# yzqin/s4g-release

Hardware: AMD Instinct MI355X
Metric: scenes/sec (25.6k-pt clouds) end-to-end grasp inference (higher is better)
Workload: dtype f32 (f16x2 split)

## Files before the change

### s4g_release_amd/csrc/mlp_common.h

```cpp
#pragma once
#include "s4g_common.h"

namespace s4g {

typedef float f32x16 __attribute__((ext_vector_type(16)));
typedef __bf16 bf16x8 __attribute__((ext_vector_type(8)));
typedef _Float16 f16x8 __attribute__((ext_vector_type(8)));
typedef _Float16 f16x2 __attribute__((ext_vector_type(2)));

__device__ __forceinline__ uint32_t cvt_pk_bf16(float lo, float hi) {
  uint32_t r;
  asm("v_cvt_pk_bf16_f32 %0, %1, %2" : "=v"(r) : "v"(lo), "v"(hi));
  return r;
}


__device__ __forceinline__ uint32_t pack_h2(float a, float b) {
  f16x2 v;
  v.x = (_Float16)a;
  v.y = (_Float16)b;
  return __builtin_bit_cast(uint32_t, v);
}

__device__ __forceinline__ void split_quad_h2(float x0, float x1, float x2, float x3, float s0, float s1, float s2, float s3,
// ... 55 lines not shown

__device__ __forceinline__ float amax_rows(const float* __restrict__ slots, int lane, int p_lo, int p_hi,
                                           int rps) {
  const int s0 = rps > 0 ? p_lo / rps : 0, s1 = rps > 0 ? p_hi / rps : 0;
  float m = amax_slots(slots + (size_t)s0 * 64, lane);
  for (int sc = s0 + 1; sc <= s1; ++sc) m = fmaxf(m, amax_slots(slots + (size_t)sc * 64, lane));
  return m;
}
__device__ __forceinline__ void amax_publish(uint32_t* __restrict__ slots, uint32_t wm, int slot, int p_lo,
                                             int p_hi, int rps) {
  const int s0 = rps > 0 ? p_lo / rps : 0, s1 = rps > 0 ? p_hi / rps : 0;
  for (int sc = s0; sc <= s1; ++sc) atomicMax(slots + (size_t)sc * 64 + (slot & 63), wm);
}


typedef float f32x4 __attribute__((ext_vector_type(4)));
__device__ __forceinline__ float4 nt_load4(const float* p) {
  const f32x4 v = __builtin_nontemporal_load(reinterpret_cast<const f32x4*>(p));
  return make_float4(v.x, v.y, v.z, v.w);
}

struct WRef {
  __amdgpu_buffer_rsrc_t r;
  uint32_t off;
};
__device__ __forceinline__ WRef wref(const void* base, size_t off) {
  return WRef{__builtin_amdgcn_make_buffer_rsrc(const_cast<void*>(base), 0, 0x7FFFFFFF, 0x00020000), (uint32_t)off};
}
__device__ __forceinline__ WRef operator+(const WRef& w, size_t bytes) { return WRef{w.r, w.off + (uint32_t)bytes}; }
__device__ __forceinline__ uint4 wref_load(const WRef& w, uint32_t lane_off, uint32_t byte_off) {
  return __builtin_bit_cast(uint4, __builtin_amdgcn_raw_buffer_load_b128(w.r, (int)lane_off, (int)(w.off + byte_off), 0));
}

template <int PL>
__device__ __forceinline__ f32x16 chain_mfma(const uint4 a, const uint4 b, const f32x16 c) {
  if constexpr (PL == 2)
    return __builtin_amdgcn_mfma_f32_32x32x16_f16(__builtin_bit_cast(f16x8, a), __builtin_bit_cast(f16x8, b), c, 0, 0, 0);
  else
    return __builtin_amdgcn_mfma_f32_32x32x16_bf16(__builtin_bit_cast(bf16x8, a), __builtin_bit_cast(bf16x8, b), c, 0, 0, 0);
}

}
```

### s4g_release_amd/csrc/mlp_gemm.hip

```cpp
#include <stdlib.h>

#include "mlp_common.h"

#include <type_traits>

#ifndef S4G_CHAIN_ABLATE
#define S4G_CHAIN_ABLATE 0
#endif

namespace s4g {


constexpr int GM_BM = 128;
constexpr int GM_BN = 128;
constexpr int GM_BK = 32;
constexpr int GM_LDS = 36;
constexpr int GM_THREADS = 256;

enum { LOAD_PLAIN = 0, LOAD_GATHER = 1, LOAD_INTERP = 2, LOAD_GATHER_MLP1 = 3, LOAD_GATHER_ADD = 4,
       LOAD_INTERP_ADD = 5, LOAD_CHANNEL_FIRST = 6,
       LOAD_REL_MLP1 = 64,
       LOAD_ADD_MFMA0 = 65 };
enum { EPI_STORE = 0, EPI_MAX = 1, EPI_CHANNEL_FIRST = 2, EPI_MAX_CF = 3 };

struct GemmParams {
  int P, Cin, Kpad, Cout, relu;
  const float* W;
  const float* bias;
  const float* A;
  int lda, a_coff, a_gcol;
  int aL;
  const int* gidx;
  const float* feat;
  const float* xyz;
  const float* ctr;
  int Cf, N, M, K;
  int nscenes;
  const float4* mlp1;
  const float4* rel4;
  const int* seg4;
  const int* seg_rows;
  float* out2;
  int ldc2, split_n;
  uint32_t* out_amax2;
  const int* nidx;
  const float* nw;
  const float* sparse;
  const float* dense;
  int C2, C1, N2, N1;
  float* out;
  int ldc, c_coff, c_gcol;
  int w_gstride, b_gstride;
  float* cf_ptr[4];
  int cf_start[5];
  int cf_sigmoid_from;
// ... 882 lines not shown
    const unsigned sb_ = gridDim.x >= 1024 ? blockIdx.x - gridDim.x / 2 : blockIdx.x;    \
    if (threadIdx.x == 0 && sb_ < 512u && blockIdx.y == 0)                                 \
      g_chain_stamps[sb_ * 16 + (i)] = __builtin_amdgcn_s_memtime();                      \
  } while (0)
#else
#define S4G_STAMP(i)
#endif
constexpr int GF_RING_F16X2 = 2;
#ifndef S4G_CHAIN_RING1
#define S4G_CHAIN_RING1 2
#endif
#ifndef S4G_CHAIN_BF16_NRB
#define S4G_CHAIN_BF16_NRB 4
#endif

template <int LOADER, int EPI2, int RW, int KC, int PL>
__global__ __launch_bounds__(RW == 8 ? 512 : 256, (PL == 1 && RW != 8 && S4G_CHAIN_BF16_NRB == 2) ? 3 : 2) void mlp_chain_kernel(const GemmParams p) {
  constexpr int GF_RING = PL == 2 ? GF_RING_F16X2 : S4G_CHAIN_RING1;
  constexpr int NRB = PL == 1 ? S4G_CHAIN_BF16_NRB : 2, WROWS = 32 * NRB;
  constexpr int CW = RW == 8 ? 8 : 4 / RW, RWN = RW == 8 ? 1 : RW;
  constexpr int BM = WROWS * RWN, K = 64 * CW, NW = RWN * CW;
  constexpr int RS = 8 * NW, RPT = BM / RS;
  constexpr int astr = K + 8, aplane = BM * astr, KS = K >> 4;
  extern __shared__ __attribute__((aligned(16))) float smemf[];
  uint16_t* Ah = reinterpret_cast<uint16_t*>(smemf);
  float* scr = reinterpret_cast<float*>(Ah + PL * aplane);
  const int g = blockIdx.y;

  const int t = threadIdx.x;
  const int lane = t & 63;
  const int wave = t >> 6;

  constexpr bool ADD0 = LOADER == LOAD_ADD_MFMA0;
  constexpr bool ADD_BOUNDS = LOADER == LOAD_GATHER_ADD || LOADER == LOAD_INTERP_ADD || ADD0;
  constexpr bool MFMA0 = LOADER == LOAD_REL_MLP1;
  static_assert(!(MFMA0 || ADD0) || (PL == 2 && KC == 1), "phase 0 on the matrix cores: f16x2, one panel");
  static_assert(!ADD0 || EPI2 == EPI_MAX, "a wave's 64 rows are one centroid's neighbours");
  constexpr bool SEGMAX = (LOADER == LOAD_GATHER_MLP1 || MFMA0) && EPI2 == EPI_MAX;
  const int tile = blockIdx.x;
  const int p0 = tile * BM;
  bool seg_scene = false;
  if constexpr (SEGMAX) {
    if (p.seg_rows) {
      const int sc = p0 / p.rps;
      const int nrows = p.seg_rows[sc];
      if (p0 - sc * p.rps >= nrows) return;
      seg_scene = nrows < p.rps;
    }
  }
  const int p_hi = min(p0 + BM, p.P) - 1;
  const int am_s0 = p.rps > 0 ? p0 / p.rps : 0, am_s1 = p.rps > 0 ? p_hi / p.rps : 0;
  float am_v1 = 0.f, am_v2 = 0.f;
  if (PL == 2 && p.a_amax) am_v1 = p.a_amax[(size_t)am_s0 * 64 + lane];
  if (PL == 2 && p.a_amax2) am_v2 = p.a_amax2[(size_t)am_s0 * 64 + lane];

  const int wr = wave / CW, wc = wave % CW;
  const int li = lane & 31, lh = lane >> 5;
  const int wc_u = __builtin_amdgcn_readfirstlane(wc);
  const uint32_t wf_lane = (uint32_t)lane * 16u;
  constexpr size_t cb_stride = (size_t)KS * PL * 1024;
  constexpr size_t strip_stride = (size_t)CW * 2 * cb_stride;
  constexpr int kchunks = KC;
  const size_t cbs1 = (size_t)kchunks * cb_stride;
  const WRef w1 = wref(p.Wfrag + (size_t)g * p.Cout * p.Kpad16 * PL, (size_t)(wc_u * 2) * cbs1);
  const bool tri = p.Wfrag3 != nullptr;
  const WRef wmid = wref(p.Wfrag2 + (size_t)g * p.Cout2 * K * PL, (size_t)(wc_u * 2) * cb_stride);
  const int CoutF = tri ? p.Cout3 : p.Cout2;
  const float* __restrict__ scF = PL == 2 ? (tri ? p.w_inv_scale3 : p.w_inv_scale2) + (size_t)g * CoutF : nullptr;
  const float* __restrict__ bgF = (tri ? p.bias3 : p.bias2) + (size_t)g * CoutF;
  const WRef w2 = tri ? wref(p.Wfrag3 + (size_t)g * CoutF * K * PL, (size_t)(wc_u * 2) * cb_stride) : wmid;
  const int nstrip2 = (CoutF + 64 * CW - 1) / (64 * CW);
  const bool active0 = wc_u * 64 < CoutF;

  uint4 ring[GF_RING][2][PL];
#pragma unroll
  for (int d = 0; d < GF_RING; ++d)
#pragma unroll
    for (int cb = 0; cb < 2; ++cb)
#pragma unroll
      for (int pl = 0; pl < PL; ++pl)
        ring[d][cb][pl] = wref_load(w1, wf_lane + pl * 1024, (uint32_t)(cb * cbs1 + (size_t)d * PL * 1024));

  S4G_STAMP(0);
  ALoader<LOADER, RPT, RS> ld;
  float4 rv0[NRB];
  float4 wv0 = f4zero();
  constexpr int NKT0 = ADD0 ? K / 32 : 1, RPT0 = ADD0 ? RPT : 1;
  float4 fa[NKT0][RPT0];
  constexpr int fstr = K + 4;
  if constexpr (ADD0) {
    const int rows_left = p.P - p0;
    const __amdgpu_buffer_rsrc_t ridx = __builtin_amdgcn_make_buffer_rsrc(
        const_cast<int*>(p.gidx + p0), 0, (rows_left < BM ? rows_left : BM) * 4, 0x00020000);
    const __amdgpu_buffer_rsrc_t rxyz = __builtin_amdgcn_make_buffer_rsrc(
        const_cast<float*>(p.xyz), 0, p.nscenes * 3 * p.N * 4, 0x00020000);
    const __amdgpu_buffer_rsrc_t rfeat = __builtin_amdgcn_make_buffer_rsrc(
        const_cast<float*>(p.feat), 0, p.nscenes * p.N * p.Cf * 4, 0x00020000);
    constexpr uint32_t OOB = 0x80000000u;
    int jr[NRB], jg[RPT];
#pragma unroll
    for (int rb = 0; rb < NRB; ++rb)
      jr[rb] = __builtin_amdgcn_raw_buffer_load_b32(ridx, (wr * WROWS + rb * 32 + li) * 4, 0, 0);
#pragma unroll
    for (int s = 0; s < RPT; ++s) jg[s] = __builtin_amdgcn_raw_buffer_load_b32(ridx, ((t >> 3) + RS * s) * 4, 0, 0);
    {
      int bw, mw;
      gather_row_bm(p.M, p.K, p0, __builtin_amdgcn_readfirstlane(wr * WROWS), bw, mw);
      bw = __builtin_amdgcn_readfirstlane(bw);
      mw = __builtin_amdgcn_readfirstlane(mw);
      const bool okw = p0 + wr * WROWS < p.P;
      float cx = 0.f, cy = 0.f, cz = 0.f;
      if (okw) {
        const float* c = p.ctr + (size_t)bw * 3 * p.M + mw;
        cx = c[0];
        cy = c[p.M];
        cz = c[2 * p.M];
      }
// ... 12 lines not shown
    for (int s = 0; s < RPT; ++s) {
      const int c64 = (RS * s) / 64 * 64;
      int bc, mc;
      gather_row_bm(p.M, p.K, p0, c64, bc, mc);
      bc = __builtin_amdgcn_readfirstlane(bc);
      rowoff[s] = p0 + c64 < p.P ? (uint32_t)((bc * p.N + jg[s]) * p.Cf + (t & 7) * 4) * 4u : OOB;
    }
    if (p.Cin >= K) {
#pragma unroll
      for (int kt = 0; kt < NKT0; ++kt)
#pragma unroll
        for (int s = 0; s < RPT; ++s)
          fa[kt][s] = __builtin_bit_cast(float4, __builtin_amdgcn_raw_buffer_load_b128(rfeat, rowoff[s] + kt * 128, 0, 0));
    } else {
#pragma unroll
      for (int kt = 0; kt < NKT0; ++kt)
#pragma unroll
        for (int s = 0; s < RPT; ++s)
          fa[kt][s] = __builtin_bit_cast(float4, __builtin_amdgcn_raw_buffer_load_b128(
                                                     rfeat, kt * 32 + (t & 7) * 4 < p.Cin ? rowoff[s] + kt * 128 : OOB, 0, 0));
    }
    const int ch = wc * 64 + lane;
    if (ch < p.Cin) wv0 = p.mlp1[ch];
  } else if constexpr (MFMA0) {
    const int rows_left = p.P - p0;
    const __amdgpu_buffer_rsrc_t rrel = __builtin_amdgcn_make_buffer_rsrc(
        const_cast<float4*>(p.rel4 + p0), 0, (rows_left < BM ? rows_left : BM) * 16, 0x00020000);
#pragma unroll
    for (int rb = 0; rb < NRB; ++rb)
      rv0[rb] = __builtin_bit_cast(float4, __builtin_amdgcn_raw_buffer_load_b128(
                                               rrel, (wr * WROWS + rb * 32 + li) * 16, 0, 0));
    const int ch = wc * 64 + lane;
    if (ch < p.Cin) wv0 = p.mlp1[ch];
  } else {
    ld.init(p, p0, g, t);
  }
  S4G_STAMP(1);
  float amax = PL == 2 ? p.a_amax_floor : 1.f;
  if (PL == 2 && p.a_amax) {
    float m = __uint_as_float(wave_max_u32(__float_as_uint(am_v1)));
    for (int sc = am_s0 + 1; sc <= am_s1; ++sc) m = fmaxf(m, amax_slots(p.a_amax + (size_t)sc * 64, lane));
    amax = ADD_BOUNDS ? amax + m : fmaxf(amax, m);
  }
  if (PL == 2 && p.a_amax2) {
    float m = __uint_as_float(wave_max_u32(__float_as_uint(am_v2)));
    for (int sc = am_s0 + 1; sc <= am_s1; ++sc) m = fmaxf(m, amax_slots(p.a_amax2 + (size_t)sc * 64, lane));
    amax = ADD_BOUNDS ? amax + m : fmaxf(amax, m);
  }
  uint32_t ex = __float_as_uint(amax) >> 23;
  ex = ex < 15u ? 15u : (ex > 240u ? 240u : ex);
  ex = __builtin_amdgcn_readfirstlane(ex);
  const float sa = PL == 2 ? __uint_as_float((268u - ex) << 23) : 1.f;
  const float inv_sa = PL == 2 ? __uint_as_float((ex - 14u) << 23) : 1.f;
  auto load_panel = [&](int kc, auto depth_tag) {
    constexpr int DEPTH = decltype(depth_tag)::value;
    const int chunk = t & 7, srow = t >> 3;
    constexpr int NKT = K / 32;
#pragma unroll
    for (int kt0 = 0; kt0 < NKT; kt0 += DEPTH) {
      float4 ra[DEPTH][RPT];
#pragma unroll
      for (int kt = 0; kt < DEPTH; ++kt)
#pragma unroll
        for (int s = 0; s < RPT; ++s) ra[kt][s] = ld.load(p, s, kc * K + (kt0 + kt) * 32 + chunk * 4, t);
#pragma unroll
      for (int kt = 0; kt < DEPTH; ++kt)
#pragma unroll
        for (int s = 0; s < RPT; ++s) {
          uint16_t* dst = Ah + (srow + RS * s) * astr + (kt0 + kt) * 32 + chunk * 4;
          if constexpr (PL == 2) {
            uint2 h, l;
            split2_h<false>(ra[kt][s], sa, h, l);
            *reinterpret_cast<uint2*>(dst) = h;
            *reinterpret_cast<uint2*>(dst + aplane) = l;
          } else {
            *reinterpret_cast<uint2*>(dst) = make_uint2(cvt_pk_bf16(ra[kt][s].x, ra[kt][s].y),
                                                        cvt_pk_bf16(ra[kt][s].z, ra[kt][s].w));
          }
        }
      if (DEPTH < NKT) __builtin_amdgcn_sched_barrier(0);
    }
  };
  const uint16_t* a_lane = Ah + (wr * WROWS + li) * astr + 8 * lh;
  float* epi_s = scr + wave * 128;
  f32x16 acc[2][NRB];
  if constexpr (MFMA0 || ADD0) {
    float m = 0.f;
#pragma unroll
    for (int rb = 0; rb < NRB; ++rb)
      m = fmaxf(m, fmaxf(fmaxf(fabsf(rv0[rb].x), fabsf(rv0[rb].y)), fabsf(rv0[rb].z)));
    uint32_t ea = wave_max_u32(__float_as_uint(m)) >> 23;
    ea = ea < 90u ? 90u : (ea > 240u ? 240u : ea);
    ea = __builtin_amdgcn_readfirstlane(ea);
    const float s_a = __uint_as_float((268u - ea) << 23), inv_a = __uint_as_float((ea - 14u) << 23);
    const float one = __uint_as_float((ea + 1u) << 23), inv_one = __uint_as_float((253u - ea) << 23);
    const float bq = wv0.w * inv_one;
    const float mw = fmaxf(fmaxf(fabsf(wv0.x), fabsf(wv0.y)), fmaxf(fabsf(wv0.z), fabsf(bq)));
    uint32_t ew = __float_as_uint(mw) >> 23;
    ew = ew < 15u ? 15u : (ew > 240u ? 240u : ew);
    const float s_w = __uint_as_float((268u - ew) << 23);
    epi_s[lane] = __uint_as_float((ew - 14u) << 23) * inv_a * (ADD0 ? 1.f : sa);
    uint32_t wh01, wl01, wh23, wl23;
    split_quad_h(wv0.x, wv0.y, wv0.z, bq, s_w, wh01, wl01, wh23, wl23);
    uint4 af0[NRB][2], bf0[2][2];
#pragma unroll
    for (int cb = 0; cb < 2; ++cb) {
      bf0[cb][0] = make_uint4(lh == cb ? wh01 : 0u, lh == cb ? wh23 : 0u, 0u, 0u);
      bf0[cb][1] = make_uint4(lh == cb ? wl01 : 0u, lh == cb ? wl23 : 0u, 0u, 0u);
    }
#pragma unroll
    for (int rb = 0; rb < NRB; ++rb) {
      const float one_r = p0 + wr * WROWS + rb * 32 + li < p.P ? one : 0.f;
      uint32_t h01, l01, h23, l23;
// ... 40 lines not shown
          }
        }
      __syncthreads();
#pragma unroll
      for (int nb = 0; nb < 2; ++nb)
#pragma unroll
        for (int j = 0; j < 4; ++j)
#pragma unroll
          for (int pb = 0; pb < NRB; ++pb) {
            uint16_t* dst = Ah + (wr * WROWS + pb * 32 + li) * astr + wc * 64 + nb * 32 + 8 * j + 4 * lh;
            uint2 h, l;
            split_quad_h(fmaxf(acc[nb][pb][4 * j], 0.f), fmaxf(acc[nb][pb][4 * j + 1], 0.f),
                         fmaxf(acc[nb][pb][4 * j + 2], 0.f), fmaxf(acc[nb][pb][4 * j + 3], 0.f), sa, h.x, l.x, h.y, l.y);
            *reinterpret_cast<uint2*>(dst) = h;
            *reinterpret_cast<uint2*>(dst + aplane) = l;
          }
    } else {
#pragma unroll
      for (int nb = 0; nb < 2; ++nb)
#pragma unroll
        for (int j = 0; j < 4; ++j) {
          const float4 f4 = *reinterpret_cast<const float4*>(epi_s + nb * 32 + 8 * j + 4 * lh);
#pragma unroll
          for (int pb = 0; pb < NRB; ++pb) {
            uint16_t* dst = Ah + (wr * WROWS + pb * 32 + li) * astr + wc * 64 + nb * 32 + 8 * j + 4 * lh;
            uint2 h, l;
            split_quad_h2(fmaxf(acc[nb][pb][4 * j], 0.f), fmaxf(acc[nb][pb][4 * j + 1], 0.f),
                          fmaxf(acc[nb][pb][4 * j + 2], 0.f), fmaxf(acc[nb][pb][4 * j + 3], 0.f), f4.x, f4.y, f4.z, f4.w,
                          h.x, l.x, h.y, l.y);
            *reinterpret_cast<uint2*>(dst) = h;
            *reinterpret_cast<uint2*>(dst + aplane) = l;
          }
        }
    }
  } else {
    if (!(S4G_CHAIN_ABLATE & 16)) load_panel(0, std::integral_constant<int, (K / 32) / (NRB / 2)>{});
  }
  S4G_STAMP(2);
  __syncthreads();
  S4G_STAMP(3);

  auto zero_acc = [&]() {
#pragma unroll
    for (int i = 0; i < 2; ++i)
#pragma unroll
      for (int j = 0; j < NRB; ++j)
#pragma unroll
        for (int r = 0; r < 16; ++r) acc[i][j][r] = 0.f;
  };
  uint4 afn[NRB][PL];
  auto prime_a = [&]() {
#pragma unroll
    for (int rb = 0; rb < NRB; ++rb)
#pragma unroll
      for (int pl = 0; pl < PL; ++pl)
        afn[rb][pl] = *reinterpret_cast<const uint4*>(a_lane + pl * aplane + rb * 32 * astr);
  };

#define S4G_F2_STRIP(SWAPPED, ZFIRST, wcur, cbs_cur, wnext, cbs_next)                                                     \
  _Pragma("unroll") for (int ks = 0; ks < KS; ++ks) {                                                  \
    const int d = ks % GF_RING;                                                                        \
    const int ksn = ks + 1 == KS ? 0 : ks + 1;                                                         \
    uint4 af[NRB][PL], bf[2][PL];                                                                      \
    _Pragma("unroll") for (int rb = 0; rb < NRB; ++rb) _Pragma("unroll") for (int pl = 0; pl < PL; ++pl) { \
      af[rb][pl] = afn[rb][pl];                                                                        \
      if (!(S4G_CHAIN_ABLATE & 2))                                                                     \
// ... 427 lines not shown
  if (r == 0 || Kpad16 <= 0 || Kpad16 % C) return 0;
  const int kc = Kpad16 / C;
#define S4G_FUSED2_Q(L, E, R, KCH) \
  if (loader == L && epilogue == (int)E && r == R && kc == KCH) return 1;
  S4G_FUSED2_LIST(S4G_FUSED2_Q)
#undef S4G_FUSED2_Q
  return 0;
}

extern "C" int s4g_mlp_gemm_f32(const s4g_gemm_desc_t* d, s4g_stream_t stream) {
  using namespace s4g;
  if (!d || d->P < 0 || d->Cout <= 0 || d->groups <= 0 || !d->bias) return S4G_EINVAL;
  const bool split = d->precision == S4G_GEMM_BF16X3 || d->precision == S4G_GEMM_BF16;
  const bool h2 = d->precision == S4G_GEMM_F16X2;
  if (h2) {
    if (!d->W_f16x2 || !d->w_inv_scale || d->Kpad16 <= 0 || (d->Kpad16 & 15) ||
        !(d->a_amax_floor >= 0.f) || (!d->a_amax && !d->a_amax2 && !(d->a_amax_floor > 0.f)))
      return S4G_EINVAL;
  } else if (split) {
    if (!d->W_bf16x3 || d->Kpad16 <= 0 || (d->Kpad16 & 15)) return S4G_EINVAL;
  } else if (d->precision == S4G_GEMM_FP32) {
    if (!d->W || d->Kpad <= 0 || (d->Kpad & 7)) return S4G_EINVAL;
  } else {
    return S4G_EINVAL;
  }
  if (d->P == 0) return S4G_OK;
  GemmParams p;
  p.P = d->P; p.Cin = d->Cin; p.Kpad = d->Kpad; p.Cout = d->Cout; p.relu = d->relu;
  p.W = d->W; p.bias = d->bias;
  p.A = d->A; p.lda = d->lda; p.a_coff = d->a_coff; p.a_gcol = d->a_gcol; p.aL = d->a_L;
  p.gidx = d->gidx; p.feat = d->feat; p.xyz = d->xyz; p.ctr = d->ctr;
  p.Cf = d->Cf; p.N = d->N; p.M = d->M; p.K = d->K;
  p.nscenes = d->M > 0 && d->K > 0 ? (int)((d->P + (int64_t)d->M * d->K - 1) / ((int64_t)d->M * d->K)) : 0;
  p.mlp1 = (const float4*)d->mlp1_w;
  p.rel4 = (const float4*)d->rel_xyz4;
  p.seg4 = d->seg4;
  p.seg_rows = d->seg_rows;
  p.out2 = d->out2;
  p.ldc2 = d->ldc2;
  p.split_n = d->out2 ? d->split_n : 0;
  p.out_amax2 = (uint32_t*)d->out_amax2;
  p.nidx = d->nidx; p.nw = d->nw; p.sparse = d->sparse; p.dense = d->dense;
  p.C2 = d->C2; p.C1 = d->C1; p.N2 = d->N2; p.N1 = d->N1;
  p.out = d->out; p.ldc = d->ldc; p.c_coff = d->c_coff; p.c_gcol = d->c_gcol;
  p.w_gstride = d->w_gstride; p.b_gstride = d->b_gstride;
  for (int i = 0; i < 4; ++i) p.cf_ptr[i] = d->cf_ptr[i];
  for (int i = 0; i < 5; ++i) p.cf_start[i] = d->cf_start[i];
  p.cf_sigmoid_from = d->cf_sigmoid_from; p.cf_N = d->cf_N;
  p.W3 = (const uint16_t*)d->W_bf16x3;
  p.Kpad16 = d->Kpad16;
  p.bf16_single = d->precision == S4G_GEMM_BF16 ? 1 : 0;
  p.w3_plane = (size_t)d->groups * (size_t)d->Cout * (size_t)d->Kpad16;
  p.Wh2 = (const uint16_t*)d->W_f16x2;
  p.w_inv_scale = d->w_inv_scale;
  p.a_amax = d->a_amax; p.a_amax2 = d->a_amax2; p.a_amax_floor = d->a_amax_floor;
  p.out_amax = (uint32_t*)d->out_amax;
  p.rps = d->rows_per_scene > 0 ? d->rows_per_scene : 0;
  p.Wfrag = (const uint16_t*)d->W_f16x2_frag;
  p.lbias = d->loader_bias;
  p.Wfrag2 = (const uint16_t*)d->W2_f16x2_frag;
  p.w_inv_scale2 = d->w2_inv_scale;
  p.bias2 = d->bias2;
  p.Cout2 = d->Cout2;
  p.relu2 = d->relu2;
  p.Wfrag3 = (const uint16_t*)d->W3_f16x2_frag;
  p.w_inv_scale3 = d->w3_inv_scale;
// ... 53 lines not shown
  } else if (d->epilogue == S4G_GEMM_EPI_STORE) {
    if (!d->out) return S4G_EINVAL;
  } else if (d->epilogue == S4G_GEMM_EPI_CHANNEL_FIRST) {
    if (d->cf_N <= 0 || d->groups != 1) return S4G_EINVAL;
  } else if (d->epilogue == S4G_GEMM_EPI_MAX_CHANNEL_FIRST) {
    if (d->relu != 1 || d->K < 1 || d->M < 1 || d->P % ((int64_t)d->M * d->K) || d->groups != 1 || !d->out ||
        d->W2_f16x2_frag || d->out2)
      return S4G_EINVAL;
  } else {
    return S4G_EINVAL;
  }

  if (d->W2_f16x2_frag) {
    const bool c128 = d->Cout == 128 && d->Kpad16 == 128,
               c256 = d->Cout == 256 && (d->Kpad16 == 256 || d->Kpad16 == 512 || d->Kpad16 == 1024),
               c512 = d->Cout == 512 && d->Kpad16 == 512;
    const bool store = d->epilogue == S4G_GEMM_EPI_STORE;
    const bool bf1 = d->precision == S4G_GEMM_BF16;
    if ((!h2 && !bf1) || (!store && (d->epilogue != S4G_GEMM_EPI_MAX || d->K != 64 || (d->P & 63))) ||
        (!c128 && !c256 && !c512) || d->Cout2 <= 0 || (d->Cout2 & 63) || (!store && d->groups != 1) || !d->W_f16x2_frag ||
        (d->W3_f16x2_frag && (d->Cout2 != d->Cout || d->Cout3 <= 0 || (d->Cout3 & 63) ||
                              (h2 && !d->w3_inv_scale) || !d->bias3)) ||
        (h2 && !d->w2_inv_scale) || !d->bias2 ||
        (store && (((d->ldc | d->c_coff | d->c_gcol) & 3) || ((uintptr_t)d->out & 15))))
      return S4G_EINVAL;
    if (bf1 && !store && !(d->W3_f16x2_frag ? d->relu3 : d->relu2)) return S4G_EUNSUPPORTED;
    if (h2 && d->loader == S4G_GEMM_LOAD_GATHER_MLP1 && d->rel_xyz4 && d->epilogue == S4G_GEMM_EPI_MAX &&
        d->Kpad16 == d->Cout && d->Cin <= d->Cout && (c128 || c256)) {
      const char* m0 = s4g::knob("S4G_MLP1_MFMA");
      if (!(m0 && m0[0] == '0'))
        return c128 ? launch_mlp_chain<LOAD_REL_MLP1, EPI_MAX, 2, 1, 2>(p, d->groups, st)
                    : launch_mlp_chain<LOAD_REL_MLP1, EPI_MAX, 1, 1, 2>(p, d->groups, st);
    }
    if (h2 && d->loader == S4G_GEMM_LOAD_GATHER_ADD && d->epilogue == S4G_GEMM_EPI_MAX && d->Kpad16 == d->Cout &&
        (int64_t)p.nscenes * d->N * d->Cf * 4 < (1ll << 31) && (int64_t)p.nscenes * d->N * 12 < (1ll << 31))
      return c128   ? launch_mlp_chain<LOAD_ADD_MFMA0, EPI_MAX, 2, 1, 2>(p, d->groups, st)
             : c256 ? launch_mlp_chain<LOAD_ADD_MFMA0, EPI_MAX, 1, 1, 2>(p, d->groups, st)
                    : launch_mlp_chain<LOAD_ADD_MFMA0, EPI_MAX, 8, 1, 2>(p, d->groups, st);
#define S4G_FUSED2_CASE(L, E, R, KCH)                                                        \
  if (d->loader == L && (int)d->epilogue == (int)E && (c128 ? 2 : (c256 ? 1 : 8)) == R &&     \
      d->Kpad16 / d->Cout == KCH)                                                             \
    return bf1 ? launch_mlp_chain<L, E, R, KCH, 1>(p, d->groups, st)                 \
               : launch_mlp_chain<L, E, R, KCH, 2>(p, d->groups, st);
    S4G_FUSED2_LIST(S4G_FUSED2_CASE)
#undef S4G_FUSED2_CASE
    return S4G_EUNSUPPORTED;
  }
  {
    const char* sc_env = s4g::knob("S4G_GEMM_SINGLE_CHAIN");
    const bool single_chain = !(sc_env && sc_env[0] == '0');
    const bool bf1 = d->precision == S4G_GEMM_BF16;
    const int kc = d->Kpad16 / 256;
    if (single_chain && (h2 || bf1) && d->loader == S4G_GEMM_LOAD_PLAIN && d->epilogue == S4G_GEMM_EPI_STORE &&
        d->W_f16x2_frag && d->groups == 1 && d->Cout % 256 == 0 && d->Kpad16 % 256 == 0 &&
        (kc == 1 || kc == 2 || kc == 4) && ((d->ldc | d->c_coff) & 3) == 0 && ((uintptr_t)d->out & 15) == 0 &&
        (d->Cout >= 1024 || d->Kpad16 >= 1024 || (sc_env && sc_env[0] == '1'))) {
      GemmParams q = p;
      q.Cout = 256;
      q.a_gcol = 0;
      q.c_gcol = 256;
      q.b_gstride = 256;
      const int strips = d->Cout / 256;
#define S4G_SINGLE_CASE(KCH)                                                                     \
  if (kc == KCH)                                                                                 \
    return bf1 ? launch_mlp_chain<LOAD_PLAIN, EPI_STORE, 1, KCH, 1>(q, strips, st)               \
               : launch_mlp_chain<LOAD_PLAIN, EPI_STORE, 1, KCH, 2>(q, strips, st);
// ... 60 lines not shown
```

### s4g_release_amd/csrc/mlp_heads.hip

```cpp
#include <stdlib.h>

#include "mlp_common.h"

#ifndef S4G_HEADS_ABLATE
#define S4G_HEADS_ABLATE 0
#endif

namespace s4g {

__device__ __forceinline__ void heads_keep_alive(const f32x16& v) { asm volatile("" ::"v"(v)); }

struct HeadsParams {
  int P, N;
  const float* X;
  int ldx;
  const uint16_t* W[5];
  const float* bias[5];
  const float* wsc[5];
  float* out[4];
  int ch[4];
  long long obs[4];
  int head_mask;
  int sigmoid_head;
  const float* a_amax;
  float a_floor;
  int rps;
  const uint16_t* Wp[2];
  const float* bias_p[2];
  const float* wsc_p[2];
  const int* nidx;
  const float* nw;
  const float* sparse;
  const float* dense;
  const float* lbias;
  const float* a_amax2;
  int N2;
};

template <int PL, int HD_RING, int NRBT, bool PRE>
__global__ __launch_bounds__(512, 2) void mlp_heads_kernel(const HeadsParams p) {
  constexpr int BM = 32 * NRBT, C = 256, NW = 8, astr = C + 8, aplane = BM * astr;
  constexpr int FB = PL * 1024;
  extern __shared__ __attribute__((aligned(16))) float smemf[];
  uint16_t* PA = reinterpret_cast<uint16_t*>(smemf);
  uint16_t* PB = PA + PL * aplane;
  float* scr = reinterpret_cast<float*>(PB + PL * aplane);

  const int t = threadIdx.x;
  const int lane = t & 63;
  const int li = lane & 31, lh = lane >> 5;
  const int wv = __builtin_amdgcn_readfirstlane(t >> 6);
  const int p0 = blockIdx.x * BM;
  const uint32_t wf_lane = (uint32_t)lane * 16u;

  float sa = 1.f, inv_sa = 1.f;
  if constexpr (PL == 2) {
    float amax = p.a_floor;
    if constexpr (PRE) {
      if (p.a_amax) amax += amax_rows(p.a_amax, lane, p0, min(p0 + BM, p.P) - 1, p.rps);
      if (p.a_amax2) amax += amax_rows(p.a_amax2, lane, p0, min(p0 + BM, p.P) - 1, p.rps);
    } else if (p.a_amax) {
      amax = fmaxf(amax, amax_rows(p.a_amax, lane, p0, min(p0 + BM, p.P) - 1, p.rps));
    }
    uint32_t ex = __float_as_uint(amax) >> 23;
    ex = ex < 15u ? 15u : (ex > 240u ? 240u : ex);
    ex = __builtin_amdgcn_readfirstlane(ex);
    sa = __uint_as_float((268u - ex) << 23);
    inv_sa = __uint_as_float((ex - 14u) << 23);
  }

  WRef wrs[5];
#pragma unroll
  for (int L = 0; L < 5; ++L) wrs[L] = wref(p.W[L], 0);
  auto woff = [&](int n32, int nks, int ks) { return (size_t)((n32 * nks + ks) * FB); };
  auto w0 = [&](int g, int h) { return wrs[0] + woff(g * 16 + h * 8 + wv, 16, 0); };
  auto w1 = [&](int g, int h) { return wrs[1] + woff(g * 8 + wv, 32, h * 16); };
  auto w2 = [&](int g) { return wrs[2] + woff(g * 8 + wv, 16, 0); };
  auto w3 = [&](int g) { return wrs[3] + woff(g * 4 + (wv & 3), 16, 0); };
  auto wl = [&](int g) { return wrs[4] + woff(g, 8, 0); };
  auto wload = [&](const WRef& w, uint32_t byte_off, int pl) { return wref_load(w, wf_lane + pl * 1024, byte_off); };
  const WRef wp0 = PRE ? wref(p.Wp[0], woff(wv, 16, 0)) : wrs[0];
  const WRef wp1 = PRE ? wref(p.Wp[1], woff(wv, 16, 0)) : wrs[0];

  const int hmask = p.head_mask;
  const int g_first = __builtin_ctz(hmask);
  uint4 ring[HD_RING][PL];
  {
    const WRef w = PRE ? wp0 : w0(g_first, 0);
#pragma unroll
    for (int d = 0; d < HD_RING; ++d)
#pragma unroll
      for (int pl = 0; pl < PL; ++pl) ring[d][pl] = wload(w, d * FB, pl);
  }

#pragma unroll 1
  for (int r0 = 0; r0 < BM; r0 += 64) {
    const int row = r0 + (t >> 3), chunk = t & 7;
    const bool ok = p0 + row < p.P;
    float4 ra[8];
    if constexpr (PRE) {
      const int pos = ok ? p0 + row : 0;
      const int bq = pos / p.N;
      int i3[3];
      float w3[3];
#pragma unroll
      for (int k = 0; k < 3; ++k) {
        i3[k] = bq * p.N2 + p.nidx[(size_t)pos * 3 + k];
        w3[k] = p.nw[(size_t)pos * 3 + k];
      }
#pragma unroll
      for (int h = 0; h < 2; ++h) {
        float4 a[4], b[4], c[4], y[4], bb[4];
#pragma unroll
        for (int kk = 0; kk < 4; ++kk) {
          const int col = (h * 4 + kk) * 32 + chunk * 4;
          a[kk] = *reinterpret_cast<const float4*>(p.sparse + (size_t)i3[0] * 256 + col);
          b[kk] = *reinterpret_cast<const float4*>(p.sparse + (size_t)i3[1] * 256 + col);
          c[kk] = *reinterpret_cast<const float4*>(p.sparse + (size_t)i3[2] * 256 + col);
          bb[kk] = *reinterpret_cast<const float4*>(p.lbias + col);
          y[kk] = p.dense ? *reinterpret_cast<const float4*>(p.dense + (size_t)pos * 256 + col)
                          : make_float4(0.f, 0.f, 0.f, 0.f);
        }
#pragma unroll
        for (int kk = 0; kk < 4; ++kk) {
          const float av[4] = {a[kk].x, a[kk].y, a[kk].z, a[kk].w}, bv[4] = {b[kk].x, b[kk].y, b[kk].z, b[kk].w};
          const float cv[4] = {c[kk].x, c[kk].y, c[kk].z, c[kk].w}, yv[4] = {y[kk].x, y[kk].y, y[kk].z, y[kk].w};
          const float bi[4] = {bb[kk].x, bb[kk].y, bb[kk].z, bb[kk].w};
          float r[4];
#pragma unroll
          for (int e = 0; e < 4; ++e) {
            float acc = __fmul_rn(av[e], w3[0]);
            acc = __fadd_rn(acc, __fmul_rn(bv[e], w3[1]));
            acc = __fadd_rn(acc, __fmul_rn(cv[e], w3[2]));
// ... 196 lines not shown
      const int row3 = (wv >> 2) * (BM / 2), cg = wv & 3;
      stage_sb(3, g * 128 + cg * 32, inv_sh);
      const WRef after = wv < NRBT ? wl(g) : w0(gnx, 0);
      S4G_HD_STRIP(PB, NRBT / 2, row3, w3(g), 16, after)
      panel_epilogue(half{}, row3, cg * 32);
    }
    if (wv < NRBT) {
      stage_sb(4, g * 32, inv_sh);
      S4G_HD_STRIP(PB, 1, wv * 32, wl(g), 8, w0(gnx, 0))
      const int row = p0 + wv * 32 + li;
      const int b = row / p.N, pt = row - b * p.N;
      const int nch = p.ch[g];
      float* __restrict__ base = p.out[g] + (size_t)b * (size_t)p.obs[g] + pt;
#pragma unroll
      for (int j = 0; j < 4; ++j) {
        const float4 sc4 = *reinterpret_cast<const float4*>(epi_s + 8 * j + 4 * lh);
        const float4 b4 = *reinterpret_cast<const float4*>(epi_s + 32 + 8 * j + 4 * lh);
        const float scv[4] = {sc4.x, sc4.y, sc4.z, sc4.w};
        const float bv[4] = {b4.x, b4.y, b4.z, b4.w};
#pragma unroll
        for (int e = 0; e < 4; ++e) {
          const int c = 8 * j + 4 * lh + e;
          float x = __fmaf_rn(acc[0][4 * j + e], scv[e], bv[e]);
          if (g == p.sigmoid_head) x = 1.0f / (1.0f + expf(-x));
          if (c < nch && row < p.P) base[(size_t)c * p.N] = x;
        }
      }
    }
  }
#undef S4G_HD_STRIP
#undef S4G_HD_TERM
}

template <int PL, int HD_RING, int NRBT, bool PRE>
static int launch_heads_cfg(const HeadsParams& p, hipStream_t st) {
  constexpr int BM = 32 * NRBT;
  constexpr size_t lds = sizeof(uint16_t) * 2 * PL * BM * (256 + 8) + sizeof(float) * (8 * 64 + 16);
  static_assert(lds <= 160 * 1024, "one workgroup's panels must fit a CU's LDS");
  static LdsAttrCache lds_cache;
  if (int rc = allow_dynamic_lds(reinterpret_cast<const void*>(&mlp_heads_kernel<PL, HD_RING, NRBT, PRE>), lds, lds_cache)) return rc;
  hipLaunchKernelGGL((mlp_heads_kernel<PL, HD_RING, NRBT, PRE>), dim3((unsigned)((p.P + BM - 1) / BM)), dim3(512), lds, st, p);
  S4G_LAUNCH_CHECK();
  return S4G_OK;
}
template <int PL, int HD_RING, int NRBT>
static int launch_heads(const HeadsParams& p, hipStream_t st) {
  return p.Wp[0] ? launch_heads_cfg<PL, HD_RING, NRBT, true>(p, st) : launch_heads_cfg<PL, HD_RING, NRBT, false>(p, st);
}

}

extern "C" int s4g_heads_chain_f32(const s4g_heads_desc_t* d, s4g_stream_t stream) {
  using namespace s4g;
  if (!d || d->P < 0 || d->N <= 0) return S4G_EINVAL;
  const bool pre = d->pre_W_frag[0] != nullptr;
  if (!pre && (!d->X || (d->ldx & 3) || d->ldx < 256 || ((uintptr_t)d->X & 15))) return S4G_EINVAL;
  if (pre && (!d->pre_W_frag[1] || !d->pre_bias[0] || !d->pre_bias[1] || !d->pre_nidx || !d->pre_nw ||
              !d->pre_sparse || !d->pre_lbias || d->pre_N2 < 3 || ((uintptr_t)d->pre_sparse & 15) ||
              ((uintptr_t)d->pre_dense & 15) || ((uintptr_t)d->pre_lbias & 15) ||
              (d->precision == S4G_GEMM_F16X2 && (!d->pre_w_inv_scale[0] || !d->pre_w_inv_scale[1]))))
    return S4G_EINVAL;
  if (d->precision != S4G_GEMM_F16X2 && d->precision != S4G_GEMM_BF16) return S4G_EINVAL;
  if (d->C != 256 || d->H0 != 512 || d->H1 != 256 || d->H2 != 256 || d->H3 != 128) return S4G_EUNSUPPORTED;
  HeadsParams p;
  p.P = d->P;
  p.N = d->N;
  p.X = d->X;
  p.ldx = d->ldx;
  for (int l = 0; l < 5; ++l) {
    if (!d->W_frag[l] || !d->bias[l] || (d->precision == S4G_GEMM_F16X2 && !d->w_inv_scale[l])) return S4G_EINVAL;
    p.W[l] = (const uint16_t*)d->W_frag[l];
    p.bias[l] = d->bias[l];
    p.wsc[l] = d->w_inv_scale[l];
  }
  p.head_mask = d->head_mask ? d->head_mask : 15;
  if (p.head_mask < 0 || p.head_mask > 15) return S4G_EINVAL;
  for (int h = 0; h < 4; ++h) {
    p.out[h] = nullptr;
    p.ch[h] = 0;
    p.obs[h] = 0;
    if (!((p.head_mask >> h) & 1)) continue;
    if (!d->out[h] || d->channels[h] <= 0 || d->channels[h] > 32) return S4G_EINVAL;
    p.out[h] = d->out[h];
    p.ch[h] = d->channels[h];
    if (d->out_batch_stride != 0 && d->out_batch_stride < (int64_t)d->channels[h] * d->N) return S4G_EINVAL;
    p.obs[h] = d->out_batch_stride != 0 ? (long long)d->out_batch_stride : (long long)d->channels[h] * d->N;
  }
  p.sigmoid_head = d->sigmoid_head;
  p.a_amax = d->a_amax;
  p.a_floor = d->a_amax_floor;
  p.rps = d->rows_per_scene > 0 ? d->rows_per_scene : 0;
  for (int l = 0; l < 2; ++l) {
    p.Wp[l] = pre ? (const uint16_t*)d->pre_W_frag[l] : nullptr;
    p.bias_p[l] = pre ? d->pre_bias[l] : nullptr;
    p.wsc_p[l] = pre ? d->pre_w_inv_scale[l] : nullptr;
  }
  p.nidx = pre ? d->pre_nidx : nullptr;
  p.nw = pre ? d->pre_nw : nullptr;
  p.sparse = pre ? d->pre_sparse : nullptr;
  p.dense = pre ? d->pre_dense : nullptr;
  p.lbias = pre ? d->pre_lbias : nullptr;
  p.a_amax2 = pre ? d->pre_a_amax2 : nullptr;
  p.N2 = pre ? d->pre_N2 : 0;
  if (d->precision == S4G_GEMM_F16X2 && !d->a_amax && !(d->a_amax_floor > 0.f)) return S4G_EINVAL;
  if (d->P == 0) return S4G_OK;
  hipStream_t st = (hipStream_t)stream;
  if (d->precision == S4G_GEMM_F16X2) return launch_heads<2, 4, 2>(p, st);
  return launch_heads<1, 4, 4>(p, st);
}
```

Measured before the change: 1989.

## Use buffer-resource loads for three-NN interpolation+add in chain and heads kernels

Adds an InterpRows helper that precomputes per-row buffer offsets and weights for three-neighbour feature interpolation plus skip-add and bias. It issues raw buffer loads in batches, with out-of-bounds offsets returning zeros instead of branching per element. A new LOAD_INTERP_ADD_BUF loader in the MLP chain kernel and a BUF variant of the heads kernel route through it when the offsets fit in 31 bits. The goal is to cut address arithmetic and bounds checks and to overlap more gather loads, at the cost of more live registers and extra template instantiations.

New measurement: 1985. Within noise of the previous version (-0.2%).

```diff
diff --git a/s4g_release_amd/csrc/mlp_common.h b/s4g_release_amd/csrc/mlp_common.h
--- a/s4g_release_amd/csrc/mlp_common.h
+++ b/s4g_release_amd/csrc/mlp_common.h
@@ -111,6 +111,83 @@
   return __builtin_bit_cast(uint4, __builtin_amdgcn_raw_buffer_load_b128(w.r, (int)lane_off, (int)(w.off + byte_off), 0));
 }
 
+constexpr uint32_t RSRC_OOB = 0x80000000u;
+template <int RPT>
+struct InterpRows {
+  __amdgpu_buffer_rsrc_t rs, rd, rb;
+  uint32_t so[RPT][3], dofs[RPT], bofs[RPT];
+  float w[RPT][3];
+  struct Raw {
+    float4 a, b, c, y, bb;
+  };
+
+  __device__ __forceinline__ void init(const int* nidx, const float* nw, const float* sparse, const float* dense,
+                                       const float* lbias, int P, int p0, int BM, int row0, int rstep, int n1, int n2,
+                                       int C, int cin, int c4, int sparse_rows) {
+    const int rows_left = P - p0, rows = rows_left < BM ? rows_left : BM;
+    const __amdgpu_buffer_rsrc_t ri =
+        __builtin_amdgcn_make_buffer_rsrc(const_cast<int*>(nidx + (size_t)p0 * 3), 0, rows * 12, 0x00020000);
+    const __amdgpu_buffer_rsrc_t rw =
+        __builtin_amdgcn_make_buffer_rsrc(const_cast<float*>(nw + (size_t)p0 * 3), 0, rows * 12, 0x00020000);
+    rs = __builtin_amdgcn_make_buffer_rsrc(const_cast<float*>(sparse), 0, sparse_rows * C * 4, 0x00020000);
+    rd = __builtin_amdgcn_make_buffer_rsrc(const_cast<float*>(dense ? dense + (size_t)p0 * C : nullptr), 0,
+                                           dense ? rows * C * 4 : 0, 0x00020000);
+    rb = __builtin_amdgcn_make_buffer_rsrc(const_cast<float*>(lbias), 0, cin * 4, 0x00020000);
+    int j[RPT][3];
+#pragma unroll
+    for (int s = 0; s < RPT; ++s)
+#pragma unroll
+      for (int k = 0; k < 3; ++k) {
+        j[s][k] = __builtin_amdgcn_raw_buffer_load_b32(ri, ((row0 + rstep * s) * 3 + k) * 4, 0, 0);
+        w[s][k] = __builtin_bit_cast(float, __builtin_amdgcn_raw_buffer_load_b32(rw, ((row0 + rstep * s) * 3 + k) * 4, 0, 0));
+      }
+    const int b0 = __builtin_amdgcn_readfirstlane(p0 / n1);
+#pragma unroll
+    for (int s = 0; s < RPT; ++s) {
+      const int r = row0 + rstep * s;
+      const bool live = r < rows;
+      int b = b0, rem = p0 - b0 * n1 + r;
+      while (rem >= n1) {
+        rem -= n1;
+        ++b;
+      }
+#pragma unroll
+      for (int k = 0; k < 3; ++k) so[s][k] = live ? (uint32_t)((b * n2 + j[s][k]) * C + c4) * 4u : RSRC_OOB;
+      dofs[s] = (uint32_t)(r * C + c4) * 4u;
+      bofs[s] = live ? (uint32_t)c4 * 4u : RSRC_OOB;
+    }
+  }
+
+  __device__ __forceinline__ Raw fetch(int s, int kt, bool colok) const {
+    auto ld = [&](const __amdgpu_buffer_rsrc_t& r, uint32_t off) {
+      return __builtin_bit_cast(float4, __builtin_amdgcn_raw_buffer_load_b128(r, (int)(colok ? off + kt * 128 : RSRC_OOB), 0, 0));
+    };
+    Raw v;
+    v.a = ld(rs, so[s][0]);
+    v.b = ld(rs, so[s][1]);
+    v.c = ld(rs, so[s][2]);
+    v.y = ld(rd, dofs[s]);
+    v.bb = ld(rb, bofs[s]);
+    return v;
+  }
+
+  __device__ __forceinline__ float4 finish(const Raw& v, int s) const {
+#pragma clang fp contract(off)
+    const f32x2 w0 = {w[s][0], w[s][0]}, w1 = {w[s][1], w[s][1]}, w2 = {w[s][2], w[s][2]};
+    auto half = [&](f32x2 a, f32x2 b, f32x2 c, f32x2 y, f32x2 bi) {
+      f32x2 acc = a * w0;
+      acc = acc + b * w1;
+      acc = acc + c * w2;
+      return (y + acc) + bi;
+    };
+    const f32x2 lo = half(f32x2{v.a.x, v.a.y}, f32x2{v.b.x, v.b.y}, f32x2{v.c.x, v.c.y}, f32x2{v.y.x, v.y.y},
+                          f32x2{v.bb.x, v.bb.y});
+    const f32x2 hi = half(f32x2{v.a.z, v.a.w}, f32x2{v.b.z, v.b.w}, f32x2{v.c.z, v.c.w}, f32x2{v.y.z, v.y.w},
+                          f32x2{v.bb.z, v.bb.w});
+    return make_float4(fmaxf(lo.x, 0.f), fmaxf(lo.y, 0.f), fmaxf(hi.x, 0.f), fmaxf(hi.y, 0.f));
+  }
+};
+
 template <int PL>
 __device__ __forceinline__ f32x16 chain_mfma(const uint4 a, const uint4 b, const f32x16 c) {
   if constexpr (PL == 2)
diff --git a/s4g_release_amd/csrc/mlp_gemm.hip b/s4g_release_amd/csrc/mlp_gemm.hip
--- a/s4g_release_amd/csrc/mlp_gemm.hip
+++ b/s4g_release_amd/csrc/mlp_gemm.hip
@@ -20,7 +20,8 @@
 enum { LOAD_PLAIN = 0, LOAD_GATHER = 1, LOAD_INTERP = 2, LOAD_GATHER_MLP1 = 3, LOAD_GATHER_ADD = 4,
        LOAD_INTERP_ADD = 5, LOAD_CHANNEL_FIRST = 6,
        LOAD_REL_MLP1 = 64,
-       LOAD_ADD_MFMA0 = 65 };
+       LOAD_ADD_MFMA0 = 65,
+       LOAD_INTERP_ADD_BUF = 66 };
 enum { EPI_STORE = 0, EPI_MAX = 1, EPI_CHANNEL_FIRST = 2, EPI_MAX_CF = 3 };
 
 struct GemmParams {
@@ -969,7 +970,9 @@
   const int wave = t >> 6;
 
   constexpr bool ADD0 = LOADER == LOAD_ADD_MFMA0;
-  constexpr bool ADD_BOUNDS = LOADER == LOAD_GATHER_ADD || LOADER == LOAD_INTERP_ADD || ADD0;
+  constexpr bool IADD = LOADER == LOAD_INTERP_ADD_BUF;
+  constexpr bool ADD_BOUNDS = LOADER == LOAD_GATHER_ADD || LOADER == LOAD_INTERP_ADD || ADD0 || IADD;
+  static_assert(!IADD || (KC == 1 && EPI2 == EPI_STORE), "the buffer-resource interpolation loader: one panel, stored rows");
   constexpr bool MFMA0 = LOADER == LOAD_REL_MLP1;
   static_assert(!(MFMA0 || ADD0) || (PL == 2 && KC == 1), "phase 0 on the matrix cores: f16x2, one panel");
   static_assert(!ADD0 || EPI2 == EPI_MAX, "a wave's 64 rows are one centroid's neighbours");
@@ -1019,7 +1022,8 @@
         ring[d][cb][pl] = wref_load(w1, wf_lane + pl * 1024, (uint32_t)(cb * cbs1 + (size_t)d * PL * 1024));
 
   S4G_STAMP(0);
-  ALoader<LOADER, RPT, RS> ld;
+  ALoader<IADD ? LOAD_INTERP_ADD : LOADER, RPT, RS> ld;
+  InterpRows<IADD ? RPT : 1> il;
   float4 rv0[NRB];
   float4 wv0 = f4zero();
   constexpr int NKT0 = ADD0 ? K / 32 : 1, RPT0 = ADD0 ? RPT : 1;
@@ -1098,6 +1102,9 @@
                                                rrel, (wr * WROWS + rb * 32 + li) * 16, 0, 0));
     const int ch = wc * 64 + lane;
     if (ch < p.Cin) wv0 = p.mlp1[ch];
+  } else if constexpr (IADD) {
+    il.init(p.nidx, p.nw, p.sparse, p.dense, p.lbias, p.P, p0, BM, t >> 3, RS, p.N1, p.N2, p.C2, p.Cin, (t & 7) * 4,
+            p.nscenes * p.N2);
   } else {
     ld.init(p, p0, g, t);
   }
@@ -1145,6 +1152,36 @@
           }
         }
       if (DEPTH < NKT) __builtin_amdgcn_sched_barrier(0);
+    }
+  };
+  auto load_panel_interp = [&](auto full_tag) {
+    constexpr bool FULL = decltype(full_tag)::value;
+    constexpr int NKT = K / 32, NI = NKT * RPT, IB = 4;
+    static_assert(NI % IB == 0, "whole batches");
+    const int chunk = t & 7, srow = t >> 3;
+#pragma unroll
+    for (int i0 = 0; i0 < NI; i0 += IB) {
+      typename InterpRows<IADD ? RPT : 1>::Raw raw[IB];
+#pragma unroll
+      for (int i = 0; i < IB; ++i) {
+        const int kt = (i0 + i) / RPT, s = (i0 + i) % RPT;
+        raw[i] = il.fetch(s, kt, FULL || kt * 32 + chunk * 4 < p.Cin);
+      }
+#pragma unroll
+      for (int i = 0; i < IB; ++i) {
+        const int kt = (i0 + i) / RPT, s = (i0 + i) % RPT;
+        const float4 v = il.finish(raw[i], s);
+        uint16_t* dst = Ah + (srow + RS * s) * astr + kt * 32 + chunk * 4;
+        if constexpr (PL == 2) {
+          uint2 h, l;
+          split2_h<false>(v, sa, h, l);
+          *reinterpret_cast<uint2*>(dst) = h;
+          *reinterpret_cast<uint2*>(dst + aplane) = l;
+        } else {
+          *reinterpret_cast<uint2*>(dst) = make_uint2(cvt_pk_bf16(v.x, v.y), cvt_pk_bf16(v.z, v.w));
+        }
+      }
+      __builtin_amdgcn_sched_barrier(0);
     }
   };
   const uint16_t* a_lane = Ah + (wr * WROWS + li) * astr + 8 * lh;
@@ -1251,6 +1288,13 @@
             *reinterpret_cast<uint2*>(dst + aplane) = l;
           }
         }
+    }
+  } else if constexpr (IADD) {
+    if (!(S4G_CHAIN_ABLATE & 16)) {
+      if (p.Cin >= K)
+        load_panel_interp(std::true_type{});
+      else
+        load_panel_interp(std::false_type{});
     }
   } else {
     if (!(S4G_CHAIN_ABLATE & 16)) load_panel(0, std::integral_constant<int, (K / 32) / (NRB / 2)>{});
@@ -1744,6 +1788,7 @@
   p.gidx = d->gidx; p.feat = d->feat; p.xyz = d->xyz; p.ctr = d->ctr;
   p.Cf = d->Cf; p.N = d->N; p.M = d->M; p.K = d->K;
   p.nscenes = d->M > 0 && d->K > 0 ? (int)((d->P + (int64_t)d->M * d->K - 1) / ((int64_t)d->M * d->K)) : 0;
+  if (d->loader == S4G_GEMM_LOAD_INTERP_ADD && d->N1 > 0) p.nscenes = (int)((d->P + (int64_t)d->N1 - 1) / d->N1);
   p.mlp1 = (const float4*)d->mlp1_w;
   p.rel4 = (const float4*)d->rel_xyz4;
   p.seg4 = d->seg4;
@@ -1863,6 +1908,14 @@
         return c128 ? launch_mlp_chain<LOAD_REL_MLP1, EPI_MAX, 2, 1, 2>(p, d->groups, st)
                     : launch_mlp_chain<LOAD_REL_MLP1, EPI_MAX, 1, 1, 2>(p, d->groups, st);
     }
+    if (d->loader == S4G_GEMM_LOAD_INTERP_ADD && store && d->Kpad16 == d->Cout &&
+        (int64_t)p.nscenes * d->N2 * d->C2 * 4 < (1ll << 31))
+      return bf1 ? (c128   ? launch_mlp_chain<LOAD_INTERP_ADD_BUF, EPI_STORE, 2, 1, 1>(p, d->groups, st)
+                    : c256 ? launch_mlp_chain<LOAD_INTERP_ADD_BUF, EPI_STORE, 1, 1, 1>(p, d->groups, st)
+                           : launch_mlp_chain<LOAD_INTERP_ADD_BUF, EPI_STORE, 8, 1, 1>(p, d->groups, st))
+                 : (c128   ? launch_mlp_chain<LOAD_INTERP_ADD_BUF, EPI_STORE, 2, 1, 2>(p, d->groups, st)
+                    : c256 ? launch_mlp_chain<LOAD_INTERP_ADD_BUF, EPI_STORE, 1, 1, 2>(p, d->groups, st)
+                           : launch_mlp_chain<LOAD_INTERP_ADD_BUF, EPI_STORE, 8, 1, 2>(p, d->groups, st));
     if (h2 && d->loader == S4G_GEMM_LOAD_GATHER_ADD && d->epilogue == S4G_GEMM_EPI_MAX && d->Kpad16 == d->Cout &&
         (int64_t)p.nscenes * d->N * d->Cf * 4 < (1ll << 31) && (int64_t)p.nscenes * d->N * 12 < (1ll << 31))
       return c128   ? launch_mlp_chain<LOAD_ADD_MFMA0, EPI_MAX, 2, 1, 2>(p, d->groups, st)
diff --git a/s4g_release_amd/csrc/mlp_heads.hip b/s4g_release_amd/csrc/mlp_heads.hip
--- a/s4g_release_amd/csrc/mlp_heads.hip
+++ b/s4g_release_amd/csrc/mlp_heads.hip
@@ -35,9 +35,10 @@
   const float* lbias;
   const float* a_amax2;
   int N2;
+  int nscenes;
 };
 
-template <int PL, int HD_RING, int NRBT, bool PRE>
+template <int PL, int HD_RING, int NRBT, bool PRE, bool BUF>
 __global__ __launch_bounds__(512, 2) void mlp_heads_kernel(const HeadsParams p) {
   constexpr int BM = 32 * NRBT, C = 256, NW = 8, astr = C + 8, aplane = BM * astr;
   constexpr int FB = PL * 1024;
@@ -98,7 +99,27 @@
     const int row = r0 + (t >> 3), chunk = t & 7;
     const bool ok = p0 + row < p.P;
     float4 ra[8];
-    if constexpr (PRE) {
+    if constexpr (PRE && BUF) {
+      InterpRows<1> il;
+      il.init(p.nidx, p.nw, p.sparse, p.dense, p.lbias, p.P, p0, BM, row, 0, p.N, p.N2, 256, 256, chunk * 4,
+              p.nscenes * p.N2);
+      if (!(S4G_HEADS_ABLATE & 16)) {
+#pragma unroll
+        for (int h = 0; h < 2; ++h) {
+          InterpRows<1>::Raw raw[4];
+#pragma unroll
+          for (int kk = 0; kk < 4; ++kk) raw[kk] = il.fetch(0, h * 4 + kk, true);
+#pragma unroll
+          for (int kk = 0; kk < 4; ++kk) ra[h * 4 + kk] = il.finish(raw[kk], 0);
+        }
+      } else {
+#pragma unroll
+        for (int kt = 0; kt < 8; ++kt) {
+          const float v = 0.01f * (float)((t * 8 + kt) % 97);
+          ra[kt] = make_float4(v, 1.f - v, 0.5f * v, 0.25f);
+        }
+      }
+    } else if constexpr (PRE) {
       const int pos = ok ? p0 + row : 0;
       const int bq = pos / p.N;
       int i3[3];
@@ -361,20 +382,22 @@
 #undef S4G_HD_TERM
 }
 
-template <int PL, int HD_RING, int NRBT, bool PRE>
+template <int PL, int HD_RING, int NRBT, bool PRE, bool BUF>
 static int launch_heads_cfg(const HeadsParams& p, hipStream_t st) {
   constexpr int BM = 32 * NRBT;
   constexpr size_t lds = sizeof(uint16_t) * 2 * PL * BM * (256 + 8) + sizeof(float) * (8 * 64 + 16);
   static_assert(lds <= 160 * 1024, "one workgroup's panels must fit a CU's LDS");
   static LdsAttrCache lds_cache;
-  if (int rc = allow_dynamic_lds(reinterpret_cast<const void*>(&mlp_heads_kernel<PL, HD_RING, NRBT, PRE>), lds, lds_cache)) return rc;
-  hipLaunchKernelGGL((mlp_heads_kernel<PL, HD_RING, NRBT, PRE>), dim3((unsigned)((p.P + BM - 1) / BM)), dim3(512), lds, st, p);
+  if (int rc = allow_dynamic_lds(reinterpret_cast<const void*>(&mlp_heads_kernel<PL, HD_RING, NRBT, PRE, BUF>), lds, lds_cache)) return rc;
+  hipLaunchKernelGGL((mlp_heads_kernel<PL, HD_RING, NRBT, PRE, BUF>), dim3((unsigned)((p.P + BM - 1) / BM)), dim3(512), lds, st, p);
   S4G_LAUNCH_CHECK();
   return S4G_OK;
 }
 template <int PL, int HD_RING, int NRBT>
 static int launch_heads(const HeadsParams& p, hipStream_t st) {
-  return p.Wp[0] ? launch_heads_cfg<PL, HD_RING, NRBT, true>(p, st) : launch_heads_cfg<PL, HD_RING, NRBT, false>(p, st);
+  if (!p.Wp[0]) return launch_heads_cfg<PL, HD_RING, NRBT, false, false>(p, st);
+  return (int64_t)p.nscenes * p.N2 * 1024 < (1ll << 31) ? launch_heads_cfg<PL, HD_RING, NRBT, true, true>(p, st)
+                                                        : launch_heads_cfg<PL, HD_RING, NRBT, true, false>(p, st);
 }
 
 }
@@ -431,6 +454,7 @@
   p.lbias = pre ? d->pre_lbias : nullptr;
   p.a_amax2 = pre ? d->pre_a_amax2 : nullptr;
   p.N2 = pre ? d->pre_N2 : 0;
+  p.nscenes = (int)(((int64_t)d->P + d->N - 1) / d->N);
   if (d->precision == S4G_GEMM_F16X2 && !d->a_amax && !(d->a_amax_floor > 0.f)) return S4G_EINVAL;
   if (d->P == 0) return S4G_OK;
   hipStream_t st = (hipStream_t)stream;
```
